# OzAmram/CaloDiffusion

Measured on AMD Instinct MI355X. Metric: sampled showers/sec (Dataset-2, 400-step DDIM), higher is better.
Workload: dtype f32 (convs: fp32 operands as 2-term fp16 splits on the fp16 MFMA pipe, fp32 accumulate; attention/norms fp32)

## Files before the change

### calodiffusion_amd/build.py

```python
from __future__ import annotations

import os
import subprocess
import sys
from concurrent.futures import ThreadPoolExecutor

HERE = os.path.dirname(os.path.abspath(__file__))
CSRC = os.path.join(HERE, "csrc")
LIBDIR = os.path.join(HERE, "lib")
TAG = os.environ.get("CD_BUILD_TAG", "")
LIB = os.path.join(LIBDIR, f"libcalodiff_hip{'_' + TAG if TAG else ''}.so")
SOURCES = ["kernels_conv.hip", "kernels_conv_zs.hip", "kernels_attn.hip", "kernels_conv_small.hip", "kernels_deep.hip", "kernels_wgrad16.hip", "kernels_norm_attn.hip", "kernels_misc.hip", "kernels_mlp.hip", "kernels_mlp_train.hip", "kernels_bwd.hip", "profiler.hip", "plan.hip",
           "forward.hip", "sampler.hip", "train.hip", "ops.hip", "misc_abi.hip"]
HIPCC = os.environ.get("HIPCC", "/opt/rocm/bin/hipcc")
FLAGS = ["--offload-arch=gfx950", "-O3", "-std=c++17", "-fPIC", "-fno-gpu-rdc", "-Wall", "-Wno-unused-function", "-Wno-unused-value"]
FLAGS += os.environ.get("CD_EXTRA_HIPCC_FLAGS", "").split()
FILE_FLAGS = {"kernels_conv_zs.hip": ["-mllvm", "-amdgpu-mfma-vgpr-form"]}


def _file_digest(paths, extra: str = "") -> str:
    import hashlib
    h = hashlib.sha256(extra.encode())
    for f in paths:
        h.update(os.path.basename(f).encode())
        h.update(open(f, "rb").read())
    return h.hexdigest()


def _read(path: str):
    try:
        return open(path).read().strip()
    except OSError:
        return None


def build_all(force: bool = False, verbose: bool = True) -> str:
    os.makedirs(LIBDIR, exist_ok=True)
    objdir = os.path.join(LIBDIR, "obj" + ("_" + TAG if TAG else ""))
    os.makedirs(objdir, exist_ok=True)
    inc = os.path.join(os.path.dirname(HERE), "include")
    headers = sorted(os.path.join(CSRC, f) for f in os.listdir(CSRC) if f.endswith((".h", ".inc")))
    headers += sorted(os.path.join(inc, f) for f in os.listdir(inc) if f.endswith(".h"))
    jobs = []
    objs = []
    for src in SOURCES:
        sp = os.path.join(CSRC, src)
        op = os.path.join(objdir, src.replace(".hip", ".o"))
        objs.append(op)
        flags = [*FLAGS, *FILE_FLAGS.get(os.path.basename(sp), [])]
        key = _file_digest([sp] + headers, " ".join(flags))
        if force or not os.path.exists(op) or _read(op + ".hash") != key:
            jobs.append(([HIPCC, *flags, "-c", sp, "-o", op], op, key))

    def run(cmd):
        if verbose:
            print(" ".join(cmd), flush=True)
        r = subprocess.run(cmd, capture_output=True, text=True)
        if r.returncode != 0:
            raise RuntimeError(f"hipcc failed:\n{r.stdout}\n{r.stderr}")
        if verbose and r.stderr.strip():
            print(r.stderr, file=sys.stderr)

    def compile_one(job):
        cmd, op, key = job
        if os.path.exists(op + ".hash"):
            os.remove(op + ".hash")
        run(cmd)
        with open(op + ".hash", "w") as fh:
            fh.write(key + "\n")

    with ThreadPoolExecutor(max_workers=4) as ex:
        list(ex.map(compile_one, jobs))
    want = source_hash()
    if force or jobs or not os.path.exists(LIB) or _read(LIB + ".srchash") != want:
        if os.path.exists(LIB + ".srchash"):
            os.remove(LIB + ".srchash")
        run([HIPCC, "--offload-arch=gfx950", "-shared", "-fPIC", "-o", LIB, *objs])
        with open(LIB + ".srchash", "w") as fh:
            fh.write(want + "\n")
    return LIB


def source_hash() -> str:
    import hashlib
    h = hashlib.sha256((" ".join(FLAGS) + repr(sorted(FILE_FLAGS.items()))).encode())
    inc = os.path.join(os.path.dirname(HERE), "include")
    files = [os.path.join(CSRC, f) for f in sorted(os.listdir(CSRC))] + [os.path.join(inc, f) for f in sorted(os.listdir(inc))]
    for f in files:
        if f.endswith((".hip", ".h", ".inc")):
            h.update(os.path.basename(f).encode())
            h.update(open(f, "rb").read())
    return h.hexdigest()


if __name__ == "__main__":
    print(build_all(force="--force" in sys.argv))
```

### calodiffusion_amd/csrc/cd_common.h

```cpp
#pragma once
#include <hip/hip_runtime.h>
#include <stdint.h>
#include <stddef.h>
#include <string>

typedef float f32x4 __attribute__((ext_vector_type(4)));
typedef float f32x16 __attribute__((ext_vector_type(16)));

namespace cd {

void set_error(const std::string& msg);
struct Fail {
  int code;
  std::string msg;
};
#define CD_HIP(expr)                                                                                  \
  do {                                                                                                \
    hipError_t _e = (expr);                                                                           \
    if (_e != hipSuccess)                                                                             \
      throw cd::Fail{-2, std::string(#expr) + ": " + hipGetErrorString(_e)};                          \
  } while (0)
#define CD_REQUIRE(cond, msg)                                                                         \
  do {                                                                                                \
    if (!(cond)) throw cd::Fail{-1, std::string(msg)};                                                \
// ... 52 lines not shown
  const float* coef = nullptr;
  int act = 0;
  float* ch_part = nullptr;
  int* units = nullptr;
  const void* wpk_bf16x3 = nullptr;
  int* status = nullptr;
  GnDefer defer;
  float* coef_buf = nullptr;
  const unsigned* in_absmax = nullptr;
  const float* add_src = nullptr;
  int* add_done = nullptr;
  struct GnOut {
    const float* gamma = nullptr;
    const float* beta = nullptr;
    int groups = 0;
    const float* res0 = nullptr;
    const float* res1 = nullptr;
    int res_c0 = 0;
    float* part_out = nullptr;
    int* done = nullptr;
  } gn_out;
};
struct AbsmaxWords {
  unsigned* next = nullptr;
  unsigned* end = nullptr;
  unsigned* take() {
    CD_REQUIRE(next && next < end, "internal: out of max-|x| words");
    return next++;
  }
};
const unsigned* launch_absmax_bits(const float* x, size_t n, AbsmaxWords* words, hipStream_t s);
__host__ __device__ inline void pow2_scale_for(unsigned mb, float* scale, float* inv) {
  const int e = (int)((mb >> 23) & 0xff) - 127;
  int sexp = mb == 0u ? 0 : 10 - e;
  sexp = sexp < -100 ? -100 : (sexp > 100 ? 100 : sexp);
  union { unsigned u; float f; } a, b;
  a.u = (unsigned)(127 + sexp) << 23;
  b.u = (unsigned)(127 - sexp) << 23;
  *scale = a.f;
  *inv = b.f;
}
inline size_t packed_bf16x3_bytes(int cin, int cout, int taps) {
  return (size_t)(cin / 16) * taps * ((cout + 31) / 32) * 3 * 64 * 16;
}
inline size_t packed_f16x2_bytes(int cin, int cout, int taps) {
  return (size_t)(cin / 16) * taps * ((cout + 31) / 32) * 2 * 64 * 16;
}
inline size_t packed_split16_bytes(int cin, int cout, int taps) {
  return packed_bf16x3_bytes(cin, cout, taps) + packed_f16x2_bytes(cin, cout, taps);
}
void launch_pack_weights_bf16x3(const float* w_torch, void* wpk, int cout, int cin, int taps, hipStream_t s,
                                bool transposed = false, bool flip = false);
void launch_pack_weights_f16x2(const float* w_torch, void* wpk, int cout, int cin, int taps, hipStream_t s,
                               bool transposed = false, bool flip = false);
inline void launch_pack_weights_split16(const float* w_torch, void* wpk, int cout, int cin, int taps, hipStream_t s,
                                        bool transposed = false, bool flip = false) {
  launch_pack_weights_bf16x3(w_torch, wpk, cout, cin, taps, s, transposed, flip);
  launch_pack_weights_f16x2(w_torch, (char*)wpk + packed_bf16x3_bytes(cin, cout, taps), cout, cin, taps, s, transposed, flip);
}

void launch_pack_weights(const float* w_torch, float* wpk, int cout, int cin, int taps, bool transposed, hipStream_t s,
                         bool flip = false);
void launch_pack_init_weights(const float* w_torch, float* wpk, int cout, int cin, hipStream_t s);
struct PackJob {
  const float* src;
  float* raw;
  float* pk;
  void* bf3;
  void* f16;
  int cout, cin, taps;
  int kind;
  int tr, flip;
  unsigned long long numel, n_pk, n_bf3, n_f16;
};
void launch_pack_jobs(const PackJob* d_jobs, int njobs, hipStream_t s);
void launch_pack_jobs_f16x2(const PackJob* d_jobs, int njobs, hipStream_t s);

void launch_conv_mfma(const float* in0, int c0, const float* in1, int c1, const float* wpk, const float* bias, float* out,
                      int batch, int cout, const ConvGeom& g, hipStream_t s, const ConvFusion& fu = ConvFusion());
bool try_launch_conv_zslide(const float* in0, int c0, const float* in1, int c1, const void* wpk_f16x2, const float* bias, float* out,
                            int batch, int cout, const ConvGeom& g, hipStream_t s, const ConvFusion& fu);
bool try_launch_conv_small(const float* in0, int c0, const float* in1, int c1, const void* wpk_f16x2, const float* bias, float* out,
                           int batch, int cout, const ConvGeom& g, hipStream_t s, const ConvFusion& fu);
void launch_conv_transpose_mfma(const float* in, int cin, const float* wpk, const float* bias, float* out, int batch,
                                int cout, Dims3 din, Dims3 dout, int kz, int sz, hipStream_t s,
                                const void* wpk_f16x2 = nullptr, int* status = nullptr, const unsigned* in_absmax = nullptr);

enum A_Prologue { A_NONE = 0, A_AFFINE = 1, A_SOFTMAX32 = 2, A_EXPNORM = 3 };
struct PointwiseArgs {
  const float* in0 = nullptr;
  int ld0 = 0, off0 = 0, c0 = 0;
  const float* in1 = nullptr;
  int ld1 = 0, c1 = 0;
  const float* wpk = nullptr;
  int64_t w_batch_stride = 0;
  const float* bias = nullptr;
  const float* residual = nullptr;
  float* out = nullptr;
  int batch = 0, cout = 0;
  int64_t vox = 0;
  int prologue = A_NONE;
  const float* coef = nullptr;
  int out_ld = 0, out_off = 0;
  float* ch_part = nullptr;
  const float* gn_res = nullptr;
  GnDefer gn_defer;
  const void* wpk16 = nullptr;
  int* status = nullptr;
};
inline int pointwise_units(int64_t vox) { return (int)((vox + 127) / 128); }
void launch_pointwise(const PointwiseArgs& a, hipStream_t s);

struct InitConvArgs {
  const float* x = nullptr;
  int cx = 0;
  int cin = 0;
  const float* scale_b = nullptr;
  int scale_stride = 1;
  const float* sigma_b = nullptr;
  float sigma_data = 1.f;
  const float* r_w = nullptr;
  const float* z_d = nullptr;
  const float* phi_h = nullptr;
  int use_rz = 0, use_phi = 0;
  const float* wpk = nullptr;
  const float* bias = nullptr;
  float* out = nullptr;
  int batch = 0, cout = 0;
  Dims3 dims{};
  float* coord_table = nullptr;
  bool table_ready = false;
  int* status = nullptr;
};
void launch_init_conv(const InitConvArgs& a, hipStream_t s);
void launch_init_coord_table(const InitConvArgs& a, hipStream_t s);

int gn_nsplit_for(int64_t vox, int batch);
void launch_ch_stats(const float* x, float* part, int batch, int channels, int64_t vox, int nsplit, hipStream_t s);
void launch_gn_finalize(const float* part, int units, const float* gamma, const float* beta, const float* add_bc, int add_ld,
                        float* coef, int batch, int channels, int groups, int64_t vox, hipStream_t s,
                        float* stat_out = nullptr );

size_t wgrad_partial_floats(int64_t out_vox, int batch, bool per_sample, int A, int Bc, int T);
struct WgradReduceJob {
  const float* partial;
  float* dw;
  int A, Bc, T, nslots, flags , b_total, b_off;
  unsigned first_block;
};
struct WgradReduceQueue {
  static constexpr int kMax = 80;
  WgradReduceJob job[kMax];
  int n = 0;
  unsigned blocks = 0;
};
void wgrad_queue_flush(WgradReduceQueue* q, hipStream_t s);
struct WgradAux {
  WgradReduceQueue* queue = nullptr;
  AbsmaxWords* words = nullptr;
  const unsigned* gmax = nullptr;
  const unsigned* xmax = nullptr;
};
void launch_wgrad(const float* g, int A, Dims3 dg, const float* x, int Bc, int xld, int xoff, Dims3 dx, int kd, int kh, int kw,
                  int sz, int sxy, int batch, bool per_sample, float* partial, float* dw, bool accumulate, bool transposed_out,
                  hipStream_t s, int b_total = 0, int b_off = 0,
                  const float* xcoef = nullptr, const WgradAux& aux = WgradAux());
// ... 309 lines not shown
```

### calodiffusion_amd/csrc/kernels_conv.hip

```cpp
#include "cd_common.h"
#include "split16.h"
#include "gn_defer.h"
#include <cstdio>
#include <cstdlib>
#include <cstring>
#include <algorithm>
#include <map>
#include <string>
#include <vector>

namespace cd {

static int g_conv_precision = -1;
static thread_local int tl_conv_precision_override = -1;
void set_conv_precision_override(int p) { tl_conv_precision_override = p; }
int conv_precision() {
  if (tl_conv_precision_override >= 0) return tl_conv_precision_override;
  if (g_conv_precision < 0) {
    const char* e = getenv("CD_CONV_PRECISION");
    g_conv_precision = !e ? PREC_F16X2 : (!strcmp(e, "f32") ? PREC_F32 : (!strcmp(e, "bf16x3") ? PREC_BF16X3 : PREC_F16X2));
  }
  return g_conv_precision;
}
void set_conv_precision(int p) { g_conv_precision = p; }
// ... 1538 lines not shown
      else return false;                                                     \
    } else launch_flat_inst<V, C>(a, grid, threads, lds, s);                 \
    if (a.add_src && fu.add_done) *fu.add_done = 1;                          \
    return true;                                                             \
  }
    CD_FLAT_CASE(1, 1) CD_FLAT_CASE(2, 1) CD_FLAT_CASE(3, 1) CD_FLAT_CASE(4, 1)
    CD_FLAT_CASE(1, 2) CD_FLAT_CASE(2, 2) CD_FLAT_CASE(3, 2) CD_FLAT_CASE(4, 2)
    CD_FLAT_CASE(1, 3) CD_FLAT_CASE(2, 3)
#undef CD_FLAT_CASE
    return false;
  };
  if (const char* ov = getenv("CD_FLAT_TILE")) {
    int nt, vt;
    if (sscanf(ov, "%d,%d", &nt, &vt) == 2 && nt % vt == 0 && nt / vt <= 8 && vt * CTmax <= 8 &&
        ((size_t)planes(nt) * HW + 1) * vox_bytes <= 160 * 1024 && (prec != 2 || vt * CTmax <= 4))
      return launch(nt, vt, CTmax);
  }
  static const int kCand[][2] = {{8, 2}, {4, 1}, {8, 1}, {12, 3}, {16, 2}, {16, 4}, {4, 2}, {6, 2}, {6, 3}, {2, 1},
                                 {3, 1}, {1, 1}, {2, 2}, {12, 2}, {8, 4}, {6, 1}, {3, 3}};
  struct Cand { int nt, vt, ct; };
  std::vector<Cand> cand;
  const bool small = g.out.vox() * batch <= 64 * 1024;
  for (int pass = 0; pass < (small && CTmax > 1 ? 2 : 1); ++pass) {
    const int CT = pass == 0 ? CTmax : 1;
    for (auto& c : kCand) {
      const int NT = c[0], VT = c[1];
      if (VT * CT > 8 || (CT == 3 && VT > 2)) continue;
      if (prec == 2 && VT * CT > 4) continue;
      static const bool no_extra_waves = getenv("CD_FLAT_NO_EXTRA_WAVES") != nullptr;
      const bool extra_ok = !no_extra_waves && g.out.vox() <= 128 && VT == 1 && NT <= 8;
      if ((int64_t)32 * (NT - 1) >= g.out.vox() && !extra_ok) continue;
      if (((size_t)planes(NT) * HW + 1) * vox_bytes > 150 * 1024) continue;
      if (pass == 1 && NT > 4) continue;
      cand.push_back({NT, VT, CT});
    }
  }
  if (prec == 3 && !getenv("CD_NO_WS")) {
    static const int kWs[][2] = {{8, 4}, {8, 2}, {4, 2}, {4, 4}, {8, 3}, {6, 2}, {2, 2}, {3, 1}, {1, 1}, {2, 1}};
    for (auto& c : kWs) {
      const int NMW = c[0], NLW = c[1];
      if ((int64_t)32 * (NMW - 1) >= g.out.vox()) continue;
      const size_t lds = 2 * ((size_t)planes(NMW) * HW + 1) * 96 + (size_t)NMW * CTmax * 64 * 4;
      if (lds > 160 * 1024 - 256) continue;
      cand.push_back({NMW, -NLW, CTmax});
    }
  }
  if (cand.empty()) return false;
  char key[192];
  std::snprintf(key, sizeof key, "flat%s g%d %dx%dx%d c%d+%d->%d b%d", prec == 3 ? "_bf16x3" : (prec == 2 ? "_f16x2" : "_f32"), geo,
                d.d, d.h, d.w, c0, c1, cout, batch);
  const int pick = autotune(key, (int)cand.size(), [&](int i) { launch(cand[i].nt, cand[i].vt, cand[i].ct); }, s);
  const Cand& c = cand[pick < 0 ? 0 : pick];
  return launch(c.nt, c.vt, c.ct);
}

void launch_conv_mfma(const float* in0, int c0, const float* in1, int c1, const float* wpk, const float* bias, float* out,
                      int batch, int cout, const ConvGeom& g, hipStream_t s, const ConvFusion& fu_in) {
  CD_REQUIRE((!fu_in.coef && !fu_in.defer.part) || c1 == 0, "conv: a fused input normalisation needs a single (non-concatenated) source");
  if (fu_in.units) *fu_in.units = 0;
  CD_REQUIRE(c0 % 32 == 0 && c1 % 32 == 0 && c0 > 0, "conv: channel counts must be multiples of 32");
  CD_REQUIRE(cout % 32 == 0, "conv: output channels must be a multiple of 32");
  CD_REQUIRE(g.kw <= 4, "conv: r kernel extent > 4 unsupported");
  const int CTtot = cout / 32;
  int CT = CTtot <= 3 ? CTtot : 2;
  CD_REQUIRE(CTtot % CT == 0, "conv: unsupported output channel count");
  char cat[128];
  std::snprintf(cat, sizeof cat, "conv%dx%dx%d_s%d C%d->%d @%dx%dx%d", g.kd, g.kh, g.kw, g.sh, c0 + c1, cout, g.in.d, g.in.h, g.in.w);
  const double taps = (double)g.kd * g.kh * g.kw;
  prof::Scope scope(cat, s, 2.0 * taps * (c0 + c1) * cout * (double)g.out.vox() * batch,
                    4.0 * batch * ((double)g.in.vox() * (c0 + c1) + (double)g.out.vox() * cout));
  ConvFusion fu = fu_in;
  auto materialise = [&]() {
    if (!fu.defer.part) return;
    if (fu.defer.coef_out) fu.coef_buf = fu.defer.coef_out;
    CD_REQUIRE(fu.coef_buf, "conv: deferred normalisation needs a coefficient buffer for kernels without the prologue");
    launch_gn_finalize(fu.defer.part, fu.defer.units, fu.defer.gamma, fu.defer.beta, fu.defer.add, fu.defer.add_ld, fu.coef_buf, batch,
                       fu.defer.C, fu.defer.groups, fu.defer.vox, s, fu.defer.stat_out);
    fu.coef = fu.coef_buf;
    fu.defer = GnDefer();
  };
  {
    const bool want_f32 = conv_precision() == PREC_F32, want_bf16x3 = conv_precision() == PREC_BF16X3;
    if (fu.wpk_bf16x3 && !want_f32 && !want_bf16x3 &&
        try_launch_conv_zslide(in0, c0, in1, c1, (const char*)fu.wpk_bf16x3 + packed_bf16x3_bytes(c0 + c1, cout, g.kd * g.kh * g.kw),
                               bias, out, batch, cout, g, s, fu))
      return;
    if (fu.wpk_bf16x3 && !want_f32 && !want_bf16x3 &&
        try_launch_conv_small(in0, c0, in1, c1, (const char*)fu.wpk_bf16x3 + packed_bf16x3_bytes(c0 + c1, cout, g.kd * g.kh * g.kw),
                              bias, out, batch, cout, g, s, fu))
      return;
    if (fu.wpk_bf16x3 && !want_f32 && !want_bf16x3 &&
        try_launch_conv3_flat(in0, c0, in1, c1, (const char*)fu.wpk_bf16x3 + packed_bf16x3_bytes(c0 + c1, cout, g.kd * g.kh * g.kw), bias,
                              out, batch, cout, g, s, fu, 2))
      return;
    materialise();
    if (fu.wpk_bf16x3 && !want_f32 && try_launch_conv3_flat(in0, c0, in1, c1, fu.wpk_bf16x3, bias, out, batch, cout, g, s, fu, 3))
      return;
    if (try_launch_conv3_flat(in0, c0, in1, c1, wpk, bias, out, batch, cout, g, s, fu, 0)) return;
  }
  {
    const bool want_f32 = conv_precision() == PREC_F32;
    if (fu.wpk_bf16x3 && !want_f32) {
      const bool f16_ok = conv_precision() == PREC_F16X2 && !fu.in_absmax;
      for (int pass = f16_ok ? 0 : 1; pass < 2; ++pass) {
      const bool f16 = pass == 0;
      const std::vector<ConvTile> cand3 = conv_tile_candidates(g, batch, CT, 14, f16 ? 80 : 96);
      auto launch3 = [&](const ConvTile& t) {
        ConvTiled3Args a3;
        ConvKArgs& a = a3.k;
        a3.status = fu.status;
        a.in0 = in0; a.in1 = in1; a.c0 = c0; a.c1 = c1; a.bias = bias; a.out = out;
        a.wpk = f16 ? (const float*)((const char*)fu.wpk_bf16x3 + packed_bf16x3_bytes(c0 + c1, cout, g.kd * g.kh * g.kw))
                    : (const float*)fu.wpk_bf16x3;
        a.Din = g.in.d; a.Hin = g.in.h; a.Win = g.in.w; a.Do = g.out.d; a.Ho = g.out.h; a.Wo = g.out.w;
        a.KD = g.kd; a.KH = g.kh; a.KW = g.kw; a.SZ = g.sz; a.SH = g.sh; a.SW = g.sw;
        a.TZ = t.TZ; a.TH = t.TH; a.nTZ = (g.out.d + t.TZ - 1) / t.TZ; a.nTH = (g.out.h + t.TH - 1) / t.TH;
        a.IZ = (t.TZ - 1) * g.sz + g.kd; a.IH = (t.TH - 1) * g.sh + g.kh;
        a.cout = cout; a.CTtot = CTtot; a.coef = fu.coef; a.act = fu.act;
        const int units = a.nTZ * a.nTH;
        const int64_t cap = (g.out.vox() + 31) / 32;
        a3.ch_part = (fu.ch_part && units <= cap) ? fu.ch_part : nullptr;
        if (fu.units) *fu.units = a3.ch_part ? units : 0;
        dim3 grid((unsigned)(batch * a.nTZ * a.nTH), (unsigned)(CTtot / CT));
        size_t lds = t.lds;
        const size_t red = (size_t)t.NW * CT * 32 * 2 * 4;
        if (lds < red) lds = red;
        if (f16) {
          if (t.VT == 1 && CT == 1) { launch_tiled3_inst<1, 1, 2>(a3, grid, t.NW * 64, lds, s); return; }
          if (t.VT == 2 && CT == 1) { launch_tiled3_inst<2, 1, 2>(a3, grid, t.NW * 64, lds, s); return; }
          if (t.VT == 1 && CT == 2) { launch_tiled3_inst<1, 2, 2>(a3, grid, t.NW * 64, lds, s); return; }
          CD_REQUIRE(false, "conv: no f16x2 tiled kernel instance for the chosen tiling");
        }
#define CD_T3_CASE(V, C)                                              \
  if (t.VT == V && CT == C) {                                         \
    launch_tiled3_inst<V, C>(a3, grid, t.NW * 64, lds, s);            \
    return;                                                           \
  }
        CD_T3_CASE(1, 1) CD_T3_CASE(2, 1) CD_T3_CASE(3, 1) CD_T3_CASE(4, 1)
        CD_T3_CASE(1, 2) CD_T3_CASE(2, 2) CD_T3_CASE(3, 2) CD_T3_CASE(4, 2)
        CD_T3_CASE(1, 3) CD_T3_CASE(2, 3)
#undef CD_T3_CASE
        CD_REQUIRE(false, "conv: no bf16x3 tiled kernel instance for the chosen tiling");
      };
      std::vector<ConvTile> ok;
      for (auto& t : cand3)
        if (f16 ? (t.VT * CT <= 2) : (t.VT <= 4 && !(CT == 3 && t.VT > 2))) ok.push_back(t);
      if (!ok.empty()) {
        char key3[192];
        std::snprintf(key3, sizeof key3, "tiled_%s %s b%d", f16 ? "f16x2" : "bf16x3", cat, batch);
        const int pick3 = autotune(key3, (int)ok.size(), [&](int i) { launch3(ok[i]); }, s);
        launch3(ok[pick3 < 0 ? 0 : pick3]);
        return;
      }
      }
    }
  }
  const std::vector<ConvTile> cand = conv_tile_candidates(g, batch, CT, 14);
  auto launch = [&](const ConvTile& t) {
    ConvKArgs a;
    a.in0 = in0; a.in1 = in1; a.c0 = c0; a.c1 = c1; a.wpk = wpk; a.bias = bias; a.out = out;
    a.Din = g.in.d; a.Hin = g.in.h; a.Win = g.in.w; a.Do = g.out.d; a.Ho = g.out.h; a.Wo = g.out.w;
    a.KD = g.kd; a.KH = g.kh; a.KW = g.kw; a.SZ = g.sz; a.SH = g.sh; a.SW = g.sw;
    a.TZ = t.TZ; a.TH = t.TH; a.nTZ = (g.out.d + t.TZ - 1) / t.TZ; a.nTH = (g.out.h + t.TH - 1) / t.TH;
    a.IZ = (t.TZ - 1) * g.sz + g.kd; a.IH = (t.TH - 1) * g.sh + g.kh;
    a.cout = cout; a.CTtot = CTtot; a.coef = fu.coef; a.act = fu.act;
    dim3 grid((unsigned)(batch * a.nTZ * a.nTH), (unsigned)(CTtot / CT));
// ... 283 lines not shown
      __builtin_amdgcn_sched_barrier(0);
      if (j + 1 < nstage) mfmas(s1);
      __builtin_amdgcn_sched_barrier(0);
      fetch(s1);
      __builtin_amdgcn_sched_barrier(0);
      if (j + 2 < nstage) mfmas(s2);
      __builtin_amdgcn_sched_barrier(0);
      fetch(s2);
      __builtin_amdgcn_sched_barrier(0);
      if (j + 3 < nstage) mfmas(s3);
    }
    float* tr = lds + a.tr_off + wave * (32 * 36);
#pragma unroll
    for (int ct = 0; ct < CT; ++ct) {
      const float bv = a.bias ? a.bias[ct * 32 + col] : 0.f;
#pragma unroll
      for (int r = 0; r < 16; ++r)
        tr[((r & 3) + 8 * (r >> 2) + 4 * half) * 36 + col] = (accA[ct][r] + accB[ct][r] * (1.f / 2048.f)) * ginv + bv;
      asm volatile("s_waitcnt lgkmcnt(0)" ::: "memory");
#pragma unroll
      for (int k = 0; k < 4; ++k) {
        const int row = 8 * k + (lane >> 3);
        const int off = __shfl(ooff, row, 64);
        const f32x4 q = *(const f32x4*)(tr + row * 36 + (lane & 7) * 4);
        if (off >= 0) *(f32x4*)(outb + off + ct * 32 + (lane & 7) * 4) = q;
      }
      asm volatile("s_waitcnt lgkmcnt(0)" ::: "memory");
    }
  }
  }
}

template <int CT>
static void launch_convT_inst(const ConvTArgs& a, dim3 grid, size_t lds, hipStream_t s) {
  static bool attr_set = false;
  if (!attr_set) {
    CD_HIP(hipFuncSetAttribute((const void*)conv_transpose_kernel<CT>, hipFuncAttributeMaxDynamicSharedMemorySize, 160 * 1024));
    CD_HIP(hipFuncSetAttribute((const void*)conv_transpose_f16x2_kernel<CT>, hipFuncAttributeMaxDynamicSharedMemorySize, 160 * 1024));
    attr_set = true;
  }
  if (a.wpk16) hipLaunchKernelGGL((conv_transpose_f16x2_kernel<CT>), grid, dim3(256), lds, s, a);
  else hipLaunchKernelGGL((conv_transpose_kernel<CT>), grid, dim3(256), lds, s, a);
  CD_HIP(hipGetLastError());
}

void launch_conv_transpose_mfma(const float* in, int cin, const float* wpk, const float* bias, float* out, int batch,
                                int cout, Dims3 din, Dims3 dout, int kz, int sz, hipStream_t s, const void* wpk_f16x2,
                                int* status, const unsigned* in_absmax) {
  CD_REQUIRE(cin % 32 == 0 && cout % 32 == 0, "conv_transpose: channels must be multiples of 32");
  CD_REQUIRE(sz == 1 || sz == 2, "conv_transpose: z stride must be 1 or 2");
  const bool full_range = conv_precision() != PREC_F16X2;
  ConvTArgs a;
  a.wpk16 = full_range ? nullptr : (const u32x4*)wpk_f16x2;
  a.status = status;
  a.in_absmax = in_absmax;
  a.in = in; a.cin = cin; a.wpk = wpk; a.bias = bias; a.out = out;
  a.Din = din.d; a.Hin = din.h; a.Win = din.w; a.Do = dout.d; a.Ho = dout.h; a.Wo = dout.w;
  a.KZ = kz; a.SZ = sz; a.cout = cout; a.CTtot = cout / 32;
  a.Cw = (dout.w + 1) / 2;
  a.CS = cin + LDS_VOX_PAD;
  const int Az = (dout.d + sz - 1) / sz, Bh = (dout.h + 1) / 2;
  struct TT { int tz, th; double score; };
  std::vector<TT> all;
  for (int TZ = 1; TZ <= Az; ++TZ)
    for (int TH = 1; TH <= Bh; ++TH) {
      const size_t lds = ((size_t)(TZ + 2) * (TH + 2) * din.w + 1) * a.CS * 4;
      if (lds > 140 * 1024) break;
      if (TH != Bh && (Bh + TH - 1) / TH == (Bh + TH) / (TH + 1)) continue;
      if (TZ != Az && (Az + TZ - 1) / TZ == (Az + TZ) / (TZ + 1)) continue;
      const long nblocks = (long)batch * ((Az + TZ - 1) / TZ) * ((Bh + TH - 1) / TH);
      const double ratio = (double)TZ * TH / ((double)(TZ + 2) * (TH + 2));
      const double fill = nblocks >= 512 ? 1.0 : (double)nblocks / 512.0;
      all.push_back({TZ, TH, ratio * fill});
    }
  CD_REQUIRE(!all.empty(), "conv_transpose: no tile fits in LDS");
  std::stable_sort(all.begin(), all.end(), [](const TT& x, const TT& y) { return x.score > y.score; });
  std::vector<TT> cand;
  for (size_t i = 0; i < all.size() && cand.size() < 8; ++i) cand.push_back(all[i]);
  for (size_t i = 8; i < all.size() && cand.size() < 14; i += (all.size() - 8) / 6 + 1) cand.push_back(all[i]);
  char cat[128];
  std::snprintf(cat, sizeof cat, "convT%dx4x4 C%d->%d @%dx%dx%d", kz, cin, cout, din.d, din.h, din.w);
  prof::Scope scope(cat, s, 2.0 * kz * 16 * cin * cout * (double)din.vox() * batch,
                    4.0 * batch * ((double)din.vox() * cin + (double)dout.vox() * cout));
  auto launch = [&](const TT& t) {
    ConvTArgs b = a;
    b.TZ = t.tz; b.TH = t.th;
    b.nTZ = (Az + b.TZ - 1) / b.TZ; b.nTH = (Bh + b.TH - 1) / b.TH;
    size_t lds = ((size_t)(b.TZ + 2) * (b.TH + 2) * din.w + 1) * b.CS * 4;
    if (b.wpk16) {
      lds = (lds + 15) & ~(size_t)15;
      b.tr_off = (int)(lds / 4);
      lds += 4 * 32 * 36 * 4;
    }
    dim3 grid((unsigned)(batch * b.nTZ * b.nTH));
    switch (b.CTtot) {
      case 1: launch_convT_inst<1>(b, grid, lds, s); break;
      case 2: launch_convT_inst<2>(b, grid, lds, s); break;
      case 3: launch_convT_inst<3>(b, grid, lds, s); break;
      case 4: launch_convT_inst<4>(b, grid, lds, s); break;
      default: CD_REQUIRE(false, "conv_transpose: more than 128 output channels unsupported");
    }
  };
  char key[192];
  std::snprintf(key, sizeof key, "%s k%d s%d b%d%s", cat, kz, sz, batch, a.wpk16 ? " f16x2" : "");
  const int pick = autotune(key, (int)cand.size(), [&](int i) { launch(cand[i]); }, s);
  launch(cand[pick < 0 ? 0 : pick]);
}

template <int CT, int PRO>
__global__ void __launch_bounds__(256) pointwise_kernel(PointwiseArgs a, int CTtot) {
  const int tid = threadIdx.x, lane = tid & 63, wave = tid >> 6;
  const int half = lane >> 5, col = lane & 31;
  const int b = blockIdx.y;
  const int ct0 = blockIdx.z * CT;
  const int64_t n0 = (int64_t)blockIdx.x * 128 + wave * 32;
  const int64_t n = n0 + col;
  const bool valid = n < a.vox;

  __shared__ __attribute__((aligned(16))) float sGn[128 * 4];
  __shared__ __attribute__((aligned(16))) char sGnScratch[128 * 16 + 64 * 8];
  float hv[CT][16];
  const bool full = n0 + 32 <= a.vox && (ct0 + CT) * 32 <= a.cout;
  const int rl = 4 * half;
  if (a.gn_res) {
    gn_defer_to_lds(a.gn_defer, b, sGn, sGnScratch);
    if (full) {
      const float* hp = a.gn_res + ((size_t)b * a.vox + n0) * a.cout + ct0 * 32 + col;
#pragma unroll
      for (int ct = 0; ct < CT; ++ct)
#pragma unroll
        for (int r = 0; r < 16; ++r) hv[ct][r] = hp[((r & 3) + 8 * (r >> 2) + rl) * a.cout + ct * 32];
    } else {
#pragma unroll
      for (int ct = 0; ct < CT; ++ct) {
        const int co = min((ct0 + ct) * 32 + col, a.cout - 1);
#pragma unroll
        for (int r = 0; r < 16; ++r) {
          const int64_t nr = min(n0 + (r & 3) + 8 * (r >> 2) + 4 * half, a.vox - 1);
          hv[ct][r] = a.gn_res[((size_t)b * a.vox + nr) * a.cout + co];
        }
      }
    }
  }

  f32x16 acc[CT];
#pragma unroll
  for (int ct = 0; ct < CT; ++ct)
#pragma unroll
    for (int r = 0; r < 16; ++r) acc[ct][r] = 0.f;

  const int nchunk = (a.c0 + a.c1) >> 5;
  const float* wb = a.wpk + (size_t)b * a.w_batch_stride;
  if (PRO == A_NONE && a.wpk16) {
    f32x16 accB[CT];
#pragma unroll
    for (int ct = 0; ct < CT; ++ct)
#pragma unroll
      for (int r = 0; r < 16; ++r) accB[ct][r] = 0.f;
    float amax = 0.f;
    for (int chunk = 0; chunk < nchunk; ++chunk) {
      const float* src;
      if (chunk * 32 < a.c0) src = a.in0 + ((size_t)b * a.vox + (valid ? n : 0)) * a.ld0 + a.off0 + chunk * 32 + half * 16;
      else src = a.in1 + ((size_t)b * a.vox + (valid ? n : 0)) * a.ld1 + (chunk * 32 - a.c0) + half * 16;
      f32x4 av[4];
#pragma unroll
      for (int q = 0; q < 4; ++q) {
// ... 435 lines not shown
```

Before: 90.45.

## Add z-sliding resample kernels for strided down/up 32-channel convolutions

Adds a new kernel file with specialised 32->32 channel strided downsample (3x4x4, stride 2) and transposed upsample convolutions. Each block stages input planes into an LDS ring with register double-buffering, keeps the fp16x2-split weights resident in registers, and splits taps (down) or output parity classes (up) across wavefronts. Both paths run ahead of the existing generic conv and convT paths. This targets the generic kernels' redundant halo loads and poor reuse at these shapes, at the cost of high register and LDS use with one block per CU, and grid sizing tied to the CU count.

```diff
diff --git a/calodiffusion_amd/build.py b/calodiffusion_amd/build.py
--- a/calodiffusion_amd/build.py
+++ b/calodiffusion_amd/build.py
@@ -10,12 +10,13 @@
 LIBDIR = os.path.join(HERE, "lib")
 TAG = os.environ.get("CD_BUILD_TAG", "")
 LIB = os.path.join(LIBDIR, f"libcalodiff_hip{'_' + TAG if TAG else ''}.so")
-SOURCES = ["kernels_conv.hip", "kernels_conv_zs.hip", "kernels_attn.hip", "kernels_conv_small.hip", "kernels_deep.hip", "kernels_wgrad16.hip", "kernels_norm_attn.hip", "kernels_misc.hip", "kernels_mlp.hip", "kernels_mlp_train.hip", "kernels_bwd.hip", "profiler.hip", "plan.hip",
+SOURCES = ["kernels_conv.hip", "kernels_conv_zs.hip", "kernels_conv_resample.hip", "kernels_attn.hip", "kernels_conv_small.hip", "kernels_deep.hip", "kernels_wgrad16.hip", "kernels_norm_attn.hip", "kernels_misc.hip", "kernels_mlp.hip", "kernels_mlp_train.hip", "kernels_bwd.hip", "profiler.hip", "plan.hip",
            "forward.hip", "sampler.hip", "train.hip", "ops.hip", "misc_abi.hip"]
 HIPCC = os.environ.get("HIPCC", "/opt/rocm/bin/hipcc")
 FLAGS = ["--offload-arch=gfx950", "-O3", "-std=c++17", "-fPIC", "-fno-gpu-rdc", "-Wall", "-Wno-unused-function", "-Wno-unused-value"]
 FLAGS += os.environ.get("CD_EXTRA_HIPCC_FLAGS", "").split()
-FILE_FLAGS = {"kernels_conv_zs.hip": ["-mllvm", "-amdgpu-mfma-vgpr-form"]}
+FILE_FLAGS = {"kernels_conv_zs.hip": ["-mllvm", "-amdgpu-mfma-vgpr-form"],
+              "kernels_conv_resample.hip": ["-mllvm", "-amdgpu-mfma-vgpr-form"]}
 
 
 def _file_digest(paths, extra: str = "") -> str:
diff --git a/calodiffusion_amd/csrc/cd_common.h b/calodiffusion_amd/csrc/cd_common.h
--- a/calodiffusion_amd/csrc/cd_common.h
+++ b/calodiffusion_amd/csrc/cd_common.h
@@ -158,6 +158,10 @@
                             int batch, int cout, const ConvGeom& g, hipStream_t s, const ConvFusion& fu);
 bool try_launch_conv_small(const float* in0, int c0, const float* in1, int c1, const void* wpk_f16x2, const float* bias, float* out,
                            int batch, int cout, const ConvGeom& g, hipStream_t s, const ConvFusion& fu);
+bool try_launch_conv_resample_down(const float* in0, int c0, const float* in1, int c1, const void* wpk_f16x2, const float* bias,
+                                   float* out, int batch, int cout, const ConvGeom& g, hipStream_t s, const ConvFusion& fu);
+bool try_launch_conv_resample_up(const float* in, int cin, const void* wpk_f16x2, const float* bias, float* out, int batch, int cout,
+                                 Dims3 din, Dims3 dout, int kz, int sz, hipStream_t s, int* status, const unsigned* in_absmax);
 void launch_conv_transpose_mfma(const float* in, int cin, const float* wpk, const float* bias, float* out, int batch,
                                 int cout, Dims3 din, Dims3 dout, int kz, int sz, hipStream_t s,
                                 const void* wpk_f16x2 = nullptr, int* status = nullptr, const unsigned* in_absmax = nullptr);
diff --git a/calodiffusion_amd/csrc/kernels_conv.hip b/calodiffusion_amd/csrc/kernels_conv.hip
--- a/calodiffusion_amd/csrc/kernels_conv.hip
+++ b/calodiffusion_amd/csrc/kernels_conv.hip
@@ -1644,6 +1644,10 @@
   {
     const bool want_f32 = conv_precision() == PREC_F32, want_bf16x3 = conv_precision() == PREC_BF16X3;
     if (fu.wpk_bf16x3 && !want_f32 && !want_bf16x3 &&
+        try_launch_conv_resample_down(in0, c0, in1, c1, (const char*)fu.wpk_bf16x3 + packed_bf16x3_bytes(c0 + c1, cout, g.kd * g.kh * g.kw),
+                                      bias, out, batch, cout, g, s, fu))
+      return;
+    if (fu.wpk_bf16x3 && !want_f32 && !want_bf16x3 &&
         try_launch_conv_zslide(in0, c0, in1, c1, (const char*)fu.wpk_bf16x3 + packed_bf16x3_bytes(c0 + c1, cout, g.kd * g.kh * g.kw),
                                bias, out, batch, cout, g, s, fu))
       return;
@@ -2093,6 +2097,7 @@
   std::snprintf(cat, sizeof cat, "convT%dx4x4 C%d->%d @%dx%dx%d", kz, cin, cout, din.d, din.h, din.w);
   prof::Scope scope(cat, s, 2.0 * kz * 16 * cin * cout * (double)din.vox() * batch,
                     4.0 * batch * ((double)din.vox() * cin + (double)dout.vox() * cout));
+  if (a.wpk16 && try_launch_conv_resample_up(in, cin, a.wpk16, bias, out, batch, cout, din, dout, kz, sz, s, status, in_absmax)) return;
   auto launch = [&](const TT& t) {
     ConvTArgs b = a;
     b.TZ = t.tz; b.TH = t.th;
diff --git a/calodiffusion_amd/csrc/kernels_conv_resample.hip b/calodiffusion_amd/csrc/kernels_conv_resample.hip
--- /dev/null
+++ b/calodiffusion_amd/csrc/kernels_conv_resample.hip
@@ -0,0 +1,401 @@
+#include "cd_common.h"
+#include "split16.h"
+
+#include <algorithm>
+#include <cstdlib>
+
+namespace cd {
+namespace {
+
+constexpr int RS_VB = 144;
+constexpr int RS_ZERO = 512;
+constexpr int RS_TR = 32 * 36 * 4;
+constexpr int RS_THREADS = 256;
+
+struct ResampleArgs {
+  const float* in;
+  const u32x4* wpk;
+  const float* bias;
+  float* out;
+  int D, H, W;
+  int Do, Ho, Wo;
+  int CZ;
+  int PLB;
+  int* status;
+};
+
+__device__ __forceinline__ void rs_barrier() { asm volatile("s_waitcnt lgkmcnt(0)\n\ts_barrier" ::: "memory"); }
+
+template <int NSL>
+struct PlaneStager {
+  const float* inb;
+  int HW, D, nq;
+  f32x4 v[NSL];
+  __device__ __forceinline__ void issue(int p) {
+    const bool live = p >= 0 && p < D;
+    const float* src = inb + (size_t)(live ? p : 0) * HW * 32;
+#pragma unroll
+    for (int k = 0; k < NSL; ++k) {
+      const int i = threadIdx.x + RS_THREADS * k;
+      v[k] = f32x4{0.f, 0.f, 0.f, 0.f};
+      if (live && i < nq) v[k] = *(const f32x4*)(src + (size_t)i * 4);
+    }
+  }
+  __device__ __forceinline__ void convert(char* slot, float& amax) const {
+#pragma unroll
+    for (int k = 0; k < NSL; ++k) {
+      const int i = threadIdx.x + RS_THREADS * k;
+      if (i < nq) {
+        const f32x4 x = v[k];
+        amax = fmaxf(amax, fmaxf(fmaxf(fabsf(x[0]), fabsf(x[1])), fmaxf(fabsf(x[2]), fabsf(x[3]))));
+        u32x2 t1, t2;
+        split2(x, t1, t2);
+        char* d = slot + (i >> 3) * RS_VB + ((i & 7) >> 2) * 64 + (i & 3) * 8;
+        *(u32x2*)d = t1;
+        *(u32x2*)(d + 32) = t2;
+      }
+    }
+  }
+};
+
+template <int WV, int NSL>
+__device__ __forceinline__ void down_body(const ResampleArgs& a, char* lds) {
+  constexpr int KS = WV >> 1, T0 = (WV & 1) * 24;
+  const int tid = threadIdx.x, lane = tid & 63, half = lane >> 5, col = lane & 31;
+  const int b = blockIdx.y;
+  const int HW = a.H * a.W, HWo = a.Ho * a.Wo;
+  const int z0 = blockIdx.x * a.CZ, z1 = min(z0 + a.CZ, a.Do);
+  char* const ring = lds + RS_ZERO;
+  float* const part = (float*)(ring + 5 * a.PLB);
+
+  u32x4 w1[24], w2[24];
+  {
+    const u32x4* wq = a.wpk + (size_t)(KS * 48 + T0) * 128 + lane;
+#pragma unroll
+    for (int j = 0; j < 24; ++j) {
+      w1[j] = wq[j * 128];
+      w2[j] = wq[j * 128 + 64];
+    }
+  }
+  if (tid < RS_ZERO / 4) ((float*)lds)[tid] = 0.f;
+  float amax = 0.f;
+  PlaneStager<NSL> st0, st1;
+  st0.inb = st1.inb = a.in + (size_t)b * a.D * HW * 32;
+  st0.HW = st1.HW = HW;
+  st0.D = st1.D = a.D;
+  st0.nq = st1.nq = HW * 8;
+  auto slot = [&](int p) { return ring + ((p + 1) % 5) * a.PLB; };
+  st0.issue(2 * z0 - 1);
+  st1.issue(2 * z0);
+  st0.convert(slot(2 * z0 - 1), amax);
+  st0.issue(2 * z0 + 1);
+  st1.convert(slot(2 * z0), amax);
+  st0.convert(slot(2 * z0 + 1), amax);
+  rs_barrier();
+
+  const int q = tid & 7;
+  f32x4 bq = {0.f, 0.f, 0.f, 0.f};
+  if (a.bias) bq = *(const f32x4*)(a.bias + q * 4);
+  const int ntile = (HWo + 31) >> 5;
+  const int kofs = KS * 64 + half * 16;
+  const float inv_wo = 1.f / (float)a.Wo;
+  float* const outb = a.out + (size_t)b * a.Do * HWo * 32;
+  const f32x16 zero16 = {0.f, 0.f, 0.f, 0.f, 0.f, 0.f, 0.f, 0.f, 0.f, 0.f, 0.f, 0.f, 0.f, 0.f, 0.f, 0.f};
+
+  for (int z = z0; z < z1; ++z) {
+    const bool more = z + 1 < z1;
+    if (more) {
+      st0.issue(2 * z + 2);
+      st1.issue(2 * z + 3);
+    }
+    int zb[3];
+#pragma unroll
+    for (int kz = 0; kz < 3; ++kz) zb[kz] = (int)(slot(2 * z - 1 + kz) - lds) + kofs;
+    for (int t = 0; t < ntile; ++t) {
+      const int v = t * 32 + col;
+      const bool valid = v < HWo;
+      const int vv = valid ? v : 0;
+      const int oh = (int)(((float)vv + 0.5f) * inv_wo), ow = vv - oh * a.Wo;
+      int rb[4], cb[4];
+      unsigned ok = 0;
+#pragma unroll
+      for (int k = 0; k < 4; ++k) {
+        int ih = 2 * oh - 1 + k;
+        ih = ih < 0 ? ih + a.H : (ih >= a.H ? ih - a.H : ih);
+        rb[k] = ih * a.W * RS_VB;
+        const int iw = 2 * ow - 1 + k;
+        cb[k] = iw * RS_VB;
+        if (valid && iw >= 0 && iw < a.W) ok |= 1u << k;
+      }
+      constexpr int PD = 3;
+      u32x4 fa[PD + 1][2];
+      auto load_frag = [&](int j) {
+        const int tap = T0 + j, kz = tap >> 4, kh = (tap >> 2) & 3, kw = tap & 3;
+        int addr = zb[kz] + rb[kh] + cb[kw];
+        addr = ((ok >> kw) & 1u) ? addr : (addr & 255);
+        fa[j % (PD + 1)][0] = *(const u32x4*)(lds + addr);
+        fa[j % (PD + 1)][1] = *(const u32x4*)(lds + addr + 32);
+      };
+      f32x16 A = zero16, B = zero16;
+#pragma unroll
+      for (int j = 0; j < PD; ++j) load_frag(j);
+#pragma unroll
+      for (int j = 0; j < 24; ++j) {
+        if (j + PD < 24) load_frag(j + PD);
+        __builtin_amdgcn_sched_barrier(0);
+        A = MFMA_F16(fa[j % (PD + 1)][0], w1[j], A);
+        B = MFMA_F16(fa[j % (PD + 1)][0], w2[j], B);
+        B = MFMA_F16(fa[j % (PD + 1)][1], w1[j], B);
+      }
+      float* const pt = part + (t & 1) * 4 * 32 * 36;
+#pragma unroll
+      for (int r = 0; r < 16; ++r) pt[(WV * 32 + (r & 3) + 8 * (r >> 2) + 4 * half) * 36 + col] = A[r] + B[r] * (1.f / 2048.f);
+      rs_barrier();
+      const int vo = t * 32 + (tid >> 3);
+      f32x4 s = *(const f32x4*)(pt + (tid >> 3) * 36 + q * 4);
+#pragma unroll
+      for (int w = 1; w < 4; ++w) s += *(const f32x4*)(pt + (w * 32 + (tid >> 3)) * 36 + q * 4);
+      if (vo < HWo) *(f32x4*)(outb + ((size_t)z * HWo + vo) * 32 + q * 4) = s + bq;
+    }
+    if (more) {
+      st0.convert(slot(2 * z + 2), amax);
+      st1.convert(slot(2 * z + 3), amax);
+    }
+    rs_barrier();
+  }
+  if (a.status && amax > 65504.f) atomicOr(a.status, 1);
+}
+
+template <int NSL>
+__global__ void __launch_bounds__(RS_THREADS, 1) conv_resample_down_f16x2_kernel(ResampleArgs a) {
+  extern __shared__ __attribute__((aligned(16))) char rs_lds[];
+  switch (threadIdx.x >> 6) {
+    case 0: down_body<0, NSL>(a, rs_lds); break;
+    case 1: down_body<1, NSL>(a, rs_lds); break;
+    case 2: down_body<2, NSL>(a, rs_lds); break;
+    default: down_body<3, NSL>(a, rs_lds); break;
+  }
+}
+
+template <int C, int NSL>
+__device__ __forceinline__ void up_body(const ResampleArgs& a, char* lds) {
+  constexpr int PH = C >> 1, PW = C & 1, KH0 = (PH + 1) & 1, KW0 = (PW + 1) & 1;
+  const int tid = threadIdx.x, lane = tid & 63, half = lane >> 5, col = lane & 31;
+  const int b = blockIdx.y;
+  const int HW = a.H * a.W, HWo = a.Ho * a.Wo;
+  const int nsteps = (a.Do + 1) >> 1;
+  const int j0 = blockIdx.x * a.CZ, j1 = min(j0 + a.CZ, nsteps);
+  char* const ring = lds + RS_ZERO;
+  float* const tr = (float*)(ring + 3 * a.PLB + C * RS_TR);
+
+  u32x4 w1[24], w2[24];
+#pragma unroll
+  for (int i = 0; i < 24; ++i) {
+    const int ks = i & 1, hw = (i >> 1) & 3, kz = i >> 3;
+    const int tap = (kz * 4 + KH0 + 2 * (hw >> 1)) * 4 + KW0 + 2 * (hw & 1);
+    const u32x4* wq = a.wpk + (size_t)(ks * 48 + tap) * 128 + lane;
+    w1[i] = wq[0];
+    w2[i] = wq[64];
+  }
+  if (tid < RS_ZERO / 4) ((float*)lds)[tid] = 0.f;
+  float amax = 0.f;
+  PlaneStager<NSL> st;
+  st.inb = a.in + (size_t)b * a.D * HW * 32;
+  st.HW = HW;
+  st.D = a.D;
+  st.nq = HW * 8;
+  auto slot = [&](int p) { return ring + (p % 3) * a.PLB; };
+  st.issue(j0);
+  st.convert(slot(j0), amax);
+  st.issue(j0 + 1);
+  st.convert(slot(j0 + 1), amax);
+  rs_barrier();
+
+  const int Ccnt = (a.Wo - PW + 1) >> 1;
+  const int ncls = a.H * Ccnt;
+  const int ntile = (ncls + 31) >> 5;
+  const float inv_c = 1.f / (float)Ccnt;
+  const float bv = a.bias ? a.bias[col] : 0.f;
+  float* const outb = a.out + (size_t)b * a.Do * HWo * 32;
+  const f32x16 zero16 = {0.f, 0.f, 0.f, 0.f, 0.f, 0.f, 0.f, 0.f, 0.f, 0.f, 0.f, 0.f, 0.f, 0.f, 0.f, 0.f};
+
+  auto store_tile = [&](const f32x16& A, const f32x16& B, int ooff) {
+#pragma unroll
+    for (int r = 0; r < 16; ++r) tr[((r & 3) + 8 * (r >> 2) + 4 * half) * 36 + col] = A[r] + B[r] * (1.f / 2048.f) + bv;
+    asm volatile("s_waitcnt lgkmcnt(0)" ::: "memory");
+#pragma unroll
+    for (int k = 0; k < 4; ++k) {
+      const int row = 8 * k + (lane >> 3);
+      const int off = __shfl(ooff, row, 64);
+      const f32x4 v = *(const f32x4*)(tr + row * 36 + (lane & 7) * 4);
+      if (off >= 0) *(f32x4*)(outb + (size_t)off * 32 + (lane & 7) * 4) = v;
+    }
+    asm volatile("s_waitcnt lgkmcnt(0)" ::: "memory");
+  };
+
+  for (int j = j0; j < j1; ++j) {
+    const bool more = j + 1 < j1;
+    if (more) st.issue(j + 2);
+    const int sb0 = (int)(slot(j) - lds) + half * 16, sb1 = (int)(slot(j + 1) - lds) + half * 16;
+    const bool odd_live = 2 * j + 1 < a.Do;
+    for (int t = 0; t < ntile; ++t) {
+      const int v = t * 32 + col;
+      const bool valid = v < ncls;
+      const int vv = valid ? v : 0;
+      const int bb = (int)(((float)vv + 0.5f) * inv_c), cc = vv - bb * Ccnt;
+      const int oh = 2 * bb + PH, ow = 2 * cc + PW;
+      int rb[2], cb[2];
+      unsigned ok = 0;
+#pragma unroll
+      for (int k = 0; k < 2; ++k) {
+        int ih = bb + ((PH + 1 - (KH0 + 2 * k)) >> 1);
+        ih = ih < 0 ? ih + a.H : (ih >= a.H ? ih - a.H : ih);
+        rb[k] = ih * a.W * RS_VB;
+        const int iw = cc + ((PW + 1 - (KW0 + 2 * k)) >> 1);
+        cb[k] = iw * RS_VB;
+        if (valid && iw >= 0 && iw < a.W) ok |= 1u << k;
+      }
+      const int pix = oh * a.Wo + ow;
+      for (int P = 0; P < (odd_live ? 2 : 1); ++P) {
+        auto frag = [&](int i, u32x4& x1, u32x4& x2) {
+          const int ks = i & 1, hw = (i >> 1) & 3, kz = i >> 3;
+          int addr = (kz == 0 ? sb1 : sb0) + ks * 64 + rb[hw >> 1] + cb[hw & 1];
+          addr = ((ok >> (hw & 1)) & 1u) ? addr : (addr & 255);
+          x1 = *(const u32x4*)(lds + addr);
+          x2 = *(const u32x4*)(lds + addr + 32);
+        };
+        f32x16 A = zero16, B = zero16;
+        constexpr int PD = 3;
+        u32x4 fa[PD + 1][2];
+        if (P == 0) {
+#pragma unroll
+          for (int n = 0; n < PD; ++n) frag(8 + n, fa[n][0], fa[n][1]);
+#pragma unroll
+          for (int n = 0; n < 8; ++n) {
+            if (n + PD < 8) frag(8 + n + PD, fa[(n + PD) % (PD + 1)][0], fa[(n + PD) % (PD + 1)][1]);
+            __builtin_amdgcn_sched_barrier(0);
+            A = MFMA_F16(fa[n % (PD + 1)][0], w1[8 + n], A);
+            B = MFMA_F16(fa[n % (PD + 1)][0], w2[8 + n], B);
+            B = MFMA_F16(fa[n % (PD + 1)][1], w1[8 + n], B);
+          }
+        } else {
+          auto idx = [](int n) { return n < 8 ? n : n + 8; };
+#pragma unroll
+          for (int n = 0; n < PD; ++n) frag(idx(n), fa[n][0], fa[n][1]);
+#pragma unroll
+          for (int n = 0; n < 16; ++n) {
+            if (n + PD < 16) frag(idx(n + PD), fa[(n + PD) % (PD + 1)][0], fa[(n + PD) % (PD + 1)][1]);
+            __builtin_amdgcn_sched_barrier(0);
+            A = MFMA_F16(fa[n % (PD + 1)][0], w1[idx(n)], A);
+            B = MFMA_F16(fa[n % (PD + 1)][0], w2[idx(n)], B);
+            B = MFMA_F16(fa[n % (PD + 1)][1], w1[idx(n)], B);
+          }
+        }
+        store_tile(A, B, valid ? (2 * j + P) * HWo + pix : -1);
+      }
+    }
+    if (more) st.convert(slot(j + 2), amax);
+    rs_barrier();
+  }
+  if (a.status && amax > 65504.f) atomicOr(a.status, 1);
+}
+
+template <int NSL>
+__global__ void __launch_bounds__(RS_THREADS, 1) conv_resample_up_f16x2_kernel(ResampleArgs a) {
+  extern __shared__ __attribute__((aligned(16))) char rs_lds[];
+  switch (threadIdx.x >> 6) {
+    case 0: up_body<0, NSL>(a, rs_lds); break;
+    case 1: up_body<1, NSL>(a, rs_lds); break;
+    case 2: up_body<2, NSL>(a, rs_lds); break;
+    default: up_body<3, NSL>(a, rs_lds); break;
+  }
+}
+
+constexpr size_t RS_LDS_MAX = 160 * 1024;
+constexpr int RS_MAX_NSL = 6;
+
+int rs_cus() {
+  static const int n = [] {
+    int dev = 0, cus = 0;
+    if (hipGetDevice(&dev) != hipSuccess || hipDeviceGetAttribute(&cus, hipDeviceAttributeMultiprocessorCount, dev) != hipSuccess || cus <= 0)
+      cus = 256;
+    return cus;
+  }();
+  return n;
+}
+
+void rs_chunks(int batch, int nsteps, int& nchunk, int& CZ) {
+  const int want = std::max(1, std::min(nsteps, (rs_cus() + batch - 1) / batch));
+  CZ = (nsteps + want - 1) / want;
+  nchunk = (nsteps + CZ - 1) / CZ;
+}
+
+template <int NSL>
+void rs_launch(bool up, const ResampleArgs& a, dim3 grid, size_t lds, hipStream_t s) {
+  static bool attr_set = false;
+  if (!attr_set) {
+    CD_HIP(hipFuncSetAttribute((const void*)conv_resample_down_f16x2_kernel<NSL>, hipFuncAttributeMaxDynamicSharedMemorySize, RS_LDS_MAX));
+    CD_HIP(hipFuncSetAttribute((const void*)conv_resample_up_f16x2_kernel<NSL>, hipFuncAttributeMaxDynamicSharedMemorySize, RS_LDS_MAX));
+    attr_set = true;
+  }
+  if (up) hipLaunchKernelGGL(conv_resample_up_f16x2_kernel<NSL>, grid, dim3(RS_THREADS), lds, s, a);
+  else hipLaunchKernelGGL(conv_resample_down_f16x2_kernel<NSL>, grid, dim3(RS_THREADS), lds, s, a);
+  CD_HIP(hipGetLastError());
+}
+
+bool rs_dispatch(bool up, const ResampleArgs& a, dim3 grid, size_t lds, hipStream_t s) {
+  const int nq = a.H * a.W * 8;
+  switch ((nq + RS_THREADS - 1) / RS_THREADS) {
+    case 1: rs_launch<1>(up, a, grid, lds, s); return true;
+    case 2: rs_launch<2>(up, a, grid, lds, s); return true;
+    case 3: rs_launch<3>(up, a, grid, lds, s); return true;
+    case 4: rs_launch<4>(up, a, grid, lds, s); return true;
+    case 5: rs_launch<5>(up, a, grid, lds, s); return true;
+    case 6: rs_launch<6>(up, a, grid, lds, s); return true;
+    default: return false;
+  }
+}
+
+}
+
+bool try_launch_conv_resample_down(const float* in0, int c0, const float* in1, int c1, const void* wpk_f16x2, const float* bias,
+                                   float* out, int batch, int cout, const ConvGeom& g, hipStream_t s, const ConvFusion& fu) {
+  static const bool off = getenv("CD_NO_ZS_DOWN") != nullptr;
+  if (off || !wpk_f16x2 || in1 || c1 != 0 || c0 != 32 || cout != 32) return false;
+  if (g.kd != 3 || g.kh != 4 || g.kw != 4 || g.sz != 2 || g.sh != 2 || g.sw != 2 || (g.in.h & 1)) return false;
+  if (g.out.d != (g.in.d - 1) / 2 + 1 || g.out.h != g.in.h / 2 || g.out.w != (g.in.w - 2) / 2 + 1) return false;
+  if (fu.coef || fu.defer.part || fu.ch_part || fu.in_absmax || fu.add_src || fu.gn_out.gamma) return false;
+  const int PV = g.in.h * g.in.w;
+  if ((PV * 8 + RS_THREADS - 1) / RS_THREADS > RS_MAX_NSL) return false;
+  ResampleArgs a;
+  a.in = in0; a.wpk = (const u32x4*)wpk_f16x2; a.bias = bias; a.out = out;
+  a.D = g.in.d; a.H = g.in.h; a.W = g.in.w; a.Do = g.out.d; a.Ho = g.out.h; a.Wo = g.out.w;
+  a.PLB = (PV * RS_VB + 255) & ~255;
+  a.status = fu.status;
+  const size_t lds = RS_ZERO + 5 * (size_t)a.PLB + 2 * 4 * (size_t)RS_TR;
+  if (lds > RS_LDS_MAX) return false;
+  int nchunk;
+  rs_chunks(batch, a.Do, nchunk, a.CZ);
+  return rs_dispatch(false, a, dim3((unsigned)nchunk, (unsigned)batch), lds, s);
+}
+
+bool try_launch_conv_resample_up(const float* in, int cin, const void* wpk_f16x2, const float* bias, float* out, int batch, int cout,
+                                 Dims3 din, Dims3 dout, int kz, int sz, hipStream_t s, int* status, const unsigned* in_absmax) {
+  static const bool off = getenv("CD_NO_ZS_UP") != nullptr;
+  if (off || !wpk_f16x2 || in_absmax || cin != 32 || cout != 32 || kz != 3 || sz != 2 || (din.h & 1)) return false;
+  if (dout.d != 2 * din.d - 1 || dout.h != 2 * din.h || (dout.w != 2 * din.w && dout.w != 2 * din.w + 1)) return false;
+  const int PV = din.h * din.w;
+  if ((PV * 8 + RS_THREADS - 1) / RS_THREADS > RS_MAX_NSL) return false;
+  ResampleArgs a;
+  a.in = in; a.wpk = (const u32x4*)wpk_f16x2; a.bias = bias; a.out = out;
+  a.D = din.d; a.H = din.h; a.W = din.w; a.Do = dout.d; a.Ho = dout.h; a.Wo = dout.w;
+  a.PLB = (PV * RS_VB + 255) & ~255;
+  a.status = status;
+  const size_t lds = RS_ZERO + 3 * (size_t)a.PLB + 4 * (size_t)RS_TR;
+  if (lds > RS_LDS_MAX) return false;
+  int nchunk;
+  rs_chunks(batch, (a.Do + 1) / 2, nchunk, a.CZ);
+  return rs_dispatch(true, a, dim3((unsigned)nchunk, (unsigned)batch), lds, s);
+}
+
+}
```

New measurement: 91.30 (median of 6 runs). Within noise of the previous version (+0.9%).
